# gMedAI-Lab/GAViKO

Measured on AMD Instinct MI355X. Metric: MRI volumes/sec (fwd+bwd) ViT-B/16 gaviko, 120x160x160, higher is better.
Workload: dtype bf16

## Files before the change

### gaviko_amd/csrc/gemm_bf16.hip

```cpp
#include "gemm_epilogue.hpp"

namespace gvk {

template <int BK>
__device__ __forceinline__ int swz_chunk(int row) {
  if constexpr (BK == 64) return (row >> 1) & 7;
  else return (0x78 >> (((row >> 2) & 3) * 2)) & 3;
}

template <int BM, int BN, int EPI, int BK = 64, bool DROP = false, int NS = 2, int NW = 4, bool SPLITK = false>
__global__ __launch_bounds__(64 * NW) void gemm_nt_kernel(GemmArgs p) {
  static_assert(NW == 4 || NW == 8, "4 or 8 waves");
  static_assert(!SPLITK || (NW == 4 && !DROP), "split-K is built on the 4-wave loops");
  static_assert(BK == 64, "the interleaved weight-row mapping is built for 128-byte tile rows");
  static_assert(NS >= 2 && NS <= 4, "2..4 LDS stages");
  constexpr int WM = BM / (NW / 2), WN = BN / 2;
  constexpr int MT = WM / 16, NT = WN / 16;
  constexpr int ROWB = BK * 2;
  constexpr int RPI = 1024 / ROWB;
  constexpr int CPR = ROWB / 16;
  constexpr int A_BYTES = BM * ROWB, W_BYTES = BN * ROWB, STAGE = A_BYTES + W_BYTES;
  extern __shared__ __attribute__((aligned(16))) char smem[];

  const int nwg = p.nbm * p.nbn;
  int wg;
  [[maybe_unused]] int piece = 0;
  if constexpr (SPLITK) {
    const int nu = nwg * p.ksplit;
    const int bid = blockIdx.x, xcd = bid & 7, q = nu >> 3, r = nu & 7;
    const int u = (xcd < r ? xcd * (q + 1) : r * (q + 1) + (xcd - r) * q) + (bid >> 3);
    wg = u / p.ksplit;
    piece = u - wg * p.ksplit;
  } else {
    const int bid = blockIdx.x, xcd = bid & 7, q = nwg >> 3, r = nwg & 7;
    wg = (xcd < r ? xcd * (q + 1) : r * (q + 1) + (xcd - r) * q) + (bid >> 3);
  }
  const int GROUP_M = p.group_m;
  const int gsz = GROUP_M * p.nbn;
  const int grp = wg / gsz, first_m = grp * GROUP_M;
  const int gm = min(p.nbm - first_m, GROUP_M);
  const int rem = wg - grp * gsz;
  int tile_m = first_m + rem % gm, tile_n = rem / gm;
  if (p.xcd_panels > 0) {
    tile_m = wg / p.nbn;
    tile_n = wg - tile_m * p.nbn;
  }
  const int m0 = tile_m * p.m_stride, n0 = tile_n * BN;

  const int lane = lane_id();
  const int wave = wave_id();
  const int wm = wave >> 1, wn = wave & 1;
  const int l15 = lane & 15, lq = lane >> 4;

  const bf16* __restrict__ Ag = p.A + (size_t)m0 * p.lda;
  const bf16* __restrict__ Wg = p.W + (size_t)n0 * p.ldw;
  if constexpr (SPLITK) {
    Ag += (size_t)piece * p.kt_per * BK;
    Wg += (size_t)piece * p.kt_per * BK;
  }

  auto stage = [&](int buf, int kt) {
    char* sA = smem + buf * STAGE;
    char* sW = sA + A_BYTES;
    const int k0 = kt * BK;
    const int rsub = lane / CPR, slot = lane % CPR;
#pragma unroll
    for (int r = 0; r < BM / (NW * RPI); ++r) {
      const int row = (r * NW + wave) * RPI + rsub;
      const int chunk = slot ^ swz_chunk<BK>(row);
      int srow = row;
      if constexpr (BM > 128 || 128 % BM != 0) srow = min(row, p.a_rows - 1 - m0);
      glds16(Ag + (size_t)srow * p.lda + k0 + chunk * 8, sA + (r * NW + wave) * 1024);
    }
#pragma unroll
    for (int r = 0; r < BN / (NW * RPI); ++r) {
      const int row = (r * NW + wave) * RPI + rsub;
      const int chunk = slot ^ swz_w(row);
      glds16(Wg + (size_t)row * p.ldw + k0 + chunk * 8, sW + (r * NW + wave) * 1024);
    }
  };

  f32x4 acc[MT][NT];
#pragma unroll
  for (int i = 0; i < MT; ++i)
#pragma unroll
    for (int j = 0; j < NT; ++j) acc[i][j] = f32x4{0.f, 0.f, 0.f, 0.f};

  int nt = p.K / BK;
  if constexpr (SPLITK) nt = min(p.kt_per, nt - piece * p.kt_per);
  if constexpr (BK == 64) {
#define GVK_LOAD_FRAGS(SA, SW, KS, XA, WB)                                                                  \
  {                                                                                                         \
    const int chunk_ = (KS) * 4 + lq;                                                                       \
    _Pragma("unroll") for (int i = 0; i < MT; ++i) {                                                        \
      const int row = wm * WM + i * 16 + l15;                                                               \
      XA[i] = *(const bf16x8*)((SA) + row * ROWB + ((chunk_ ^ swz_chunk<BK>(row)) << 4));                   \
    }                                                                                                       \
    _Pragma("unroll") for (int j = 0; j < NT; ++j) {                                                        \
      const int row = wn * WN + 32 * (j >> 1) + 8 * (l15 >> 2) + 4 * (j & 1) + (l15 & 3);                   \
      WB[j] = *(const bf16x8*)((SW) + row * ROWB + ((chunk_ ^ swz_w(row)) << 4));                           \
    }                                                                                                       \
  }
#define GVK_MMA(XA, WB)                                                                                      \
  _Pragma("unroll") for (int i = 0; i < MT; ++i)                                                            \
  _Pragma("unroll") for (int j = 0; j < NT; ++j)                                                            \
      acc[i][j] = __builtin_amdgcn_mfma_f32_16x16x32_bf16(WB[j], XA[i], acc[i][j], 0, 0, 0);
    bf16x8 xa0[MT], wb0[NT], xa1[MT], wb1[NT];
    constexpr int PER_TILE = BM / (NW * RPI) + BN / (NW * RPI);
    if constexpr (NS == 2) {
    stage(0, 0);
    if (nt > 1) stage(1, 1);
    if (nt > 1) __builtin_amdgcn_s_waitcnt(0x0F70 | (PER_TILE & 0xF) | ((PER_TILE >> 4) << 14));
    else __builtin_amdgcn_s_waitcnt(0x0F70);
    __builtin_amdgcn_s_barrier();
    GVK_LOAD_FRAGS(smem, smem + A_BYTES, 0, xa0, wb0)
    __builtin_amdgcn_s_waitcnt(0xC07F);
#define GVK_TILE(T, PREFETCH)                                                                               \
    {                                                                                                       \
      const int buf = (T) & 1;                                                                              \
      const char* sA = smem + buf * STAGE;                                                                  \
      const char* sW = sA + A_BYTES;                                                                        \
      GVK_LOAD_FRAGS(sA, sW, 1, xa1, wb1)                                                                   \
      __builtin_amdgcn_sched_barrier(0);                                                                    \
      GVK_MMA(xa0, wb0)                                                                                     \
      __builtin_amdgcn_sched_barrier(0);                                                                    \
      __syncthreads();     \
      if (PREFETCH) stage(buf, (T) + 2);                                                                    \
      GVK_LOAD_FRAGS(smem + (buf ^ 1) * STAGE, smem + (buf ^ 1) * STAGE + A_BYTES, 0, xa0, wb0)             \
      __builtin_amdgcn_sched_barrier(0);                                                                    \
      GVK_MMA(xa1, wb1)                                                                                     \
      __builtin_amdgcn_sched_barrier(0);                                                                    \
      __builtin_amdgcn_s_waitcnt(0xC07F);     \
    }
    int t = 0;
    for (; t < nt - 2; ++t) GVK_TILE(t, true)
    for (; t < nt; ++t) GVK_TILE(t, false)
#undef GVK_TILE
    } else {
    static_assert((NS - 1) * PER_TILE <= 63, "vmcnt is a 6-bit counter");
#pragma unroll
    for (int sgi = 0; sgi < NS; ++sgi)
      if (sgi < nt) stage(sgi, sgi);
    {
      const int ahead = min(nt, NS) - 1;
      if (ahead >= 3) __builtin_amdgcn_s_waitcnt(0x0F70 | ((3 * PER_TILE) & 0xF) | (((3 * PER_TILE) >> 4) << 14));
      else if (ahead == 2) __builtin_amdgcn_s_waitcnt(0x0F70 | ((2 * PER_TILE) & 0xF) | (((2 * PER_TILE) >> 4) << 14));
      else if (ahead == 1) __builtin_amdgcn_s_waitcnt(0x0F70 | (PER_TILE & 0xF) | ((PER_TILE >> 4) << 14));
      else __builtin_amdgcn_s_waitcnt(0x0F70);
    }
    __builtin_amdgcn_s_barrier();
    GVK_LOAD_FRAGS(smem, smem + A_BYTES, 0, xa0, wb0)
    __builtin_amdgcn_s_waitcnt(0xC07F);
#define GVK_TILE3(T, BUF, PREFETCH, AHEAD, LAST)                                                            \
    {                                                                                                       \
      const int buf = (BUF);                                                                                \
      const int nxt = buf == NS - 1 ? 0 : buf + 1;                                                          \
      const char* sA = smem + buf * STAGE;                                                                  \
      const char* sW = sA + A_BYTES;                                                                        \
      GVK_LOAD_FRAGS(sA, sW, 1, xa1, wb1)                                                                   \
      __builtin_amdgcn_sched_barrier(0);                                                                    \
      GVK_MMA(xa0, wb0)                                                                                     \
      __builtin_amdgcn_sched_barrier(0);                                                                    \
       \
      __builtin_amdgcn_s_waitcnt(0x0070 | (((AHEAD) * PER_TILE) & 0xF) | ((((AHEAD) * PER_TILE) >> 4) << 14)); \
      __builtin_amdgcn_s_barrier();                                                                         \
      if (PREFETCH) stage(buf, (T) + NS);                                                                   \
      if (!(LAST)) GVK_LOAD_FRAGS(smem + nxt * STAGE, smem + nxt * STAGE + A_BYTES, 0, xa0, wb0)            \
      __builtin_amdgcn_sched_barrier(0);                                                                    \
      GVK_MMA(xa1, wb1)                                                                                     \
      __builtin_amdgcn_sched_barrier(0);                                                                    \
      __builtin_amdgcn_s_waitcnt(0xC07F);                                                                   \
    }
    int t = 0, b = 0;
    for (; t < nt - NS; ++t) {
      GVK_TILE3(t, b, true, NS - 2, false)
      b = b == NS - 1 ? 0 : b + 1;
    }
    for (; t < nt; ++t) {
      const int r = nt - 1 - t;
      if (NS > 3 && r == 3) GVK_TILE3(t, b, false, 2, false)
      else if (r == 2) GVK_TILE3(t, b, false, 1, false)
      else if (r == 1) GVK_TILE3(t, b, false, 0, false)
      else GVK_TILE3(t, b, false, 0, true)
      b = b == NS - 1 ? 0 : b + 1;
    }
#undef GVK_TILE3
    }
#undef GVK_LOAD_FRAGS
#undef GVK_MMA
  }

  if constexpr (SPLITK) {
    const int tile_id = tile_m * p.nbn + tile_n;
    constexpr int kPiece = NW * MT * NT * 64 * 4;
    float* const base = p.sk_part + ((size_t)tile_id * p.ksplit) * kPiece;
    const __amdgpu_buffer_rsrc_t rs = __builtin_amdgcn_make_buffer_rsrc((void*)base, 0, p.ksplit * kPiece * 4, 0x00020000);
    const int off = ((wave * MT * NT) * 64 + lane) * 16;
#pragma unroll
    for (int i = 0; i < MT; ++i)
#pragma unroll
      for (int j = 0; j < NT; ++j)
        __builtin_amdgcn_raw_buffer_store_b128(__builtin_bit_cast(u32x4, acc[i][j]), rs, (piece * kPiece) * 4 + off + (i * NT + j) * 1024, 0, 16);
    int* const s_last = (int*)smem;
    asm volatile("s_waitcnt vmcnt(0)" ::: "memory");
    __syncthreads();
    if (threadIdx.x == 0) {
      const int t = __hip_atomic_fetch_add(p.sk_tick + tile_id, 1, __ATOMIC_RELAXED, __HIP_MEMORY_SCOPE_AGENT);
      const int last = (t == p.ksplit - 1) ? 1 : 0;
      if (last) {
        __builtin_amdgcn_fence(__ATOMIC_ACQUIRE, "agent");
        asm volatile("s_waitcnt vmcnt(0)" ::: "memory");
        __hip_atomic_store(p.sk_tick + tile_id, 0, __ATOMIC_RELAXED, __HIP_MEMORY_SCOPE_AGENT);
      }
      *s_last = last;
    }
    __syncthreads();
    if (!*s_last) return;
    if (p.ksplit == 2) {
      const int pc = piece ^ 1;
#pragma unroll
      for (int i = 0; i < MT; ++i)
#pragma unroll
        for (int j = 0; j < NT; ++j) acc[i][j] += *(const f32x4*)((const char*)base + (size_t)pc * kPiece * 4 + off + (i * NT + j) * 1024);
    } else {
#pragma unroll
      for (int i = 0; i < MT; ++i)
#pragma unroll
        for (int j = 0; j < NT; ++j) acc[i][j] = f32x4{0.f, 0.f, 0.f, 0.f};
      for (int pc = 0; pc < p.ksplit; ++pc) {
#pragma unroll
        for (int i = 0; i < MT; ++i)
#pragma unroll
          for (int j = 0; j < NT; ++j) acc[i][j] += *(const f32x4*)((const char*)base + (size_t)pc * kPiece * 4 + off + (i * NT + j) * 1024);
      }
    }
  }
  gemm_epilogue<EPI, DROP, MT, NT>(p, acc, m0 + wm * WM, n0 + wn * WN, l15, lq);
}

// ... 69 lines not shown
    const long t128 = (long)((a.M + 127) / 128) * (a.N / bn);
    static const int n768 = diag_env("GAVIKO_HIP_GEMM_N768") ? atoi(diag_env("GAVIKO_HIP_GEMM_N768")) : 3128;
    const int bm = (t128 >= 384) ? 128 : 64;
    tile = bm * 1000 + bn;
    if constexpr (EPI == GVK_EPI_STORE_BF16 || EPI == GVK_EPI_BIAS_GELU_BF16 || EPI == GVK_EPI_GELU_BWD_BF16) {
      static const int wide = diag_env("GAVIKO_HIP_GEMM_WIDE") ? atoi(diag_env("GAVIKO_HIP_GEMM_WIDE")) : 8;
      const long t256 = (long)((a.M + 255) / 256) * (a.N / 256);
      static const bool wide_bwd = diag_env("GAVIKO_HIP_GEMM_WIDE_BWD") == nullptr || diag_env("GAVIKO_HIP_GEMM_WIDE_BWD")[0] != '0';
      if (wide != 0 && a.N % 256 == 0 && a.drop_thresh == 0u && t256 >= wide_lo() && t256 <= 256 && (EPI != GVK_EPI_GELU_BWD_BF16 || wide_bwd))
        tile = (wide == 256 || a.K < 128) ? 256256 : 8256256;
    }
    static const long t64_hi = diag_env("GAVIKO_HIP_GEMM_T64HI") ? atol(diag_env("GAVIKO_HIP_GEMM_T64HI")) : 130;
    if (bm == 64 && bn == 128 && t128 <= 256 && a.K >= 512 && a.drop_thresh == 0u) {
      if (n768 == 3128) {
        long best = -1; int best_bm = 128;
        for (int cand : {128, 96, 64}) {
          const long tiles = (long)((a.M + cand - 1) / cand) * (a.N / 128);
          const long cost = ((tiles + 255) / 256) * (cand + 128);
          if (best < 0 || cost < best) { best = cost; best_bm = cand; }
        }
        static const int force_bm = diag_env("GAVIKO_HIP_GEMM_BM") ? atoi(diag_env("GAVIKO_HIP_GEMM_BM")) : 0;
        if (force_bm == 128 || force_bm == 96 || force_bm == 64) best_bm = force_bm;
        else if (t128 <= t64_hi && best_bm == 128) best_bm = 64;
        tile = best_bm == 64 ? 3064128 : best_bm == 96 ? 3096128 : 3128128;
      }
      else if (n768 == 128) tile = 128128;
      else if (n768 == 3064) tile = 3064128;
    }
  }
  if (a.drop_thresh != 0u) {
    if constexpr (EPI == GVK_EPI_BIAS_RES_F32 || EPI == GVK_EPI_BIAS_GELU_BF16 || EPI == GVK_EPI_GELU_BWD_BF16) {
      switch (tile) {
        case 128128: return launch_gemm<128, 128, EPI, true>(a, stream);
        case 128064: return launch_gemm<128, 64, EPI, true>(a, stream);
        case 64128: return launch_gemm<64, 128, EPI, true>(a, stream);
        case 64064: return launch_gemm<64, 64, EPI, true>(a, stream);
        default: return set_error(-2, "gvk_gemm_nt_bf16: unsupported tile %d", tile);
      }
    } else {
      return set_error(-2, "gvk_gemm_nt_bf16: drop_p > 0 is supported by BIAS_RES_F32, BIAS_GELU_BF16 and GELU_BWD_BF16 only");
    }
  }
  switch (tile) {
    case 8256256: return launch_gemm8p(a, EPI, 0, stream);
    case 7256256: return launch_gemm8p(a, EPI, 1, stream);
    case 2128128:
      if (a.sk_part == nullptr) return set_error(-2, "gvk_gemm_nt_bf16: tile 2128128 needs splitk_ws");
      return launch_gemm<128, 128, EPI, false, 2, 4, true>(a, stream);
    case 3128128: return launch_gemm<128, 128, EPI, false, 3>(a, stream);
    case 3064128: return launch_gemm<64, 128, EPI, false, 3>(a, stream);
    case 4064128:
      if (a.sk_part != nullptr) return launch_gemm<64, 128, EPI, false, 4, 4, true>(a, stream);
      return launch_gemm<64, 128, EPI, false, 4>(a, stream);
    case 3096128: return launch_gemm<96, 128, EPI, false, 3>(a, stream);
    case 256256:
      if constexpr (EPI == GVK_EPI_STORE_BF16 || EPI == GVK_EPI_BIAS_GELU_BF16 || EPI == GVK_EPI_GELU_BWD_BF16) return launch_gemm<256, 256, EPI, false, 2, 8>(a, stream);
      else return set_error(-2, "gvk_gemm_nt_bf16: the 256x256 tile is built for STORE_BF16, BIAS_GELU_BF16 and GELU_BWD_BF16");
    case 128128: return launch_gemm<128, 128, EPI>(a, stream);
    case 128064: return launch_gemm<128, 64, EPI>(a, stream);
    case 64128: return launch_gemm<64, 128, EPI>(a, stream);
    case 64064: return launch_gemm<64, 64, EPI>(a, stream);
    default: return set_error(-2, "gvk_gemm_nt_bf16: unsupported tile %d", tile);
  }
}

}

extern "C" int gvk_gemm_stat_parts(int N) { return N / 64; }

extern "C" int gvk_gemm_nt_bf16(const gvk_gemm_desc* d, void* stream) {
  using namespace gvk;
  GVK_REQUIRE(d != nullptr, "gvk_gemm_nt_bf16: null descriptor");
  GVK_REQUIRE(d->a && d->w && d->M > 0 && d->N > 0 && d->K > 0, "gvk_gemm_nt_bf16: null operand or empty shape");
  GVK_REQUIRE(d->K % 64 == 0, "gvk_gemm_nt_bf16: K=%d must be a multiple of 64", d->K);
  GVK_REQUIRE(d->N % 64 == 0, "gvk_gemm_nt_bf16: N=%d must be a multiple of 64", d->N);
  GVK_REQUIRE(d->lda >= d->K && d->ldw >= d->K && d->lda % 8 == 0 && d->ldw % 8 == 0,
              "gvk_gemm_nt_bf16: lda/ldw must be >= K and multiples of 8");
  GVK_REQUIRE(d->ldo % 8 == 0 && d->ldo >= d->N, "gvk_gemm_nt_bf16: ldo=%d must be >= N and a multiple of 8 (16-byte row pieces)", d->ldo);
  if (d->tile != 0) {
    const int bn = d->tile % 1000;
    GVK_REQUIRE(d->tile < 1000000 || d->K % 32 == 0, "gvk_gemm_nt_bf16: K not a multiple of 32");
    GVK_REQUIRE(bn > 0 && d->N % bn == 0, "gvk_gemm_nt_bf16: N=%d not a multiple of the tile's BN", d->N);
  }
  GemmArgs a{};
  a.A = (const bf16*)d->a; a.W = (const bf16*)d->w; a.out0 = d->out0; a.out1 = d->out1;
  a.bias = d->bias; a.res = d->res; a.aux = (const bf16*)d->aux; a.pos = d->pos;
  a.M = d->M; a.N = d->N; a.K = d->K; a.lda = d->lda; a.ldw = d->ldw; a.ldo = d->ldo;
  a.ldres = d->ldres; a.ldaux = d->ldaux; a.rows_in = d->rows_in; a.rows_out = d->rows_out; a.row_off = d->row_off;
  GVK_REQUIRE(d->drop_p >= 0.f && d->drop_p < 1.f && (d->drop_p == 0.f || d->seed_ptr != nullptr), "gvk_gemm_nt_bf16: drop_p in [0,1) and a seed word");
  a.seed = d->seed; a.seed_ptr = (const unsigned long long*)d->seed_ptr; a.drop_thresh = drop_threshold_u32(d->drop_p);
  a.inv_keep = d->drop_p > 0.f ? 1.f / (1.f - d->drop_p) : 1.f;
  GVK_REQUIRE(d->scale_cols == 0 || (d->epilogue == GVK_EPI_STORE_BF16 && d->scale_cols > 0 && d->scale_cols % 8 == 0 && d->scale_cols <= d->N),
              "gvk_gemm_nt_bf16: scale_cols=%d needs the STORE_BF16 epilogue, a multiple of 8 and <= N", d->scale_cols);
  a.scale_cols = d->scale_cols; a.col_scale = d->col_scale;
  GVK_REQUIRE(d->ln_mean == nullptr || (d->epilogue == GVK_EPI_STORE_BF16 && d->ln_rstd && d->ln_c1 && d->bias),
              "gvk_gemm_nt_bf16: the LayerNorm fold needs the STORE_BF16 epilogue, ln_rstd, ln_c1 and bias (= sum_c beta[c] W[n][c])");
  a.ln_mean = d->ln_mean; a.ln_rstd = d->ln_rstd; a.ln_c1 = d->ln_c1;
  GVK_REQUIRE(d->stat_part == nullptr || (d->epilogue == GVK_EPI_BIAS_RES_F32_BF16 && d->N % 128 == 0 && (d->tile == 0 || d->tile % 1000 == 128)),
              "gvk_gemm_nt_bf16: stat_part needs the BIAS_RES_F32_BF16 epilogue on 128-column tiles (64-column groups)");
  a.stat_part = d->stat_part; a.stat_pivot = d->stat_pivot;
  GVK_REQUIRE((d->m_panels == 0 && d->m_stride == 0) || (d->m_panels > 0 && d->m_stride > 0 && d->epilogue != GVK_EPI_PATCH_F32),
              "gvk_gemm_nt_bf16: m_panels=%d / m_stride=%d: both positive (or both 0), not with the PATCH epilogue", d->m_panels, d->m_stride);
  a.m_stride = d->m_stride; a.nbm = d->m_panels;
  GVK_REQUIRE(d->splitk_ws == nullptr || ((d->m_panels > 0 || d->tile == 2128128) && ((uintptr_t)d->splitk_ws & 255) == 0),
              "gvk_gemm_nt_bf16: splitk_ws goes with strided row panels or tile 2128128 (256-byte aligned)");
  GVK_REQUIRE(d->ksplit >= 0 && d->ksplit <= 8 && (d->ksplit == 0 || d->splitk_ws != nullptr), "gvk_gemm_nt_bf16: ksplit=%d: 0 (auto) .. 8, with splitk_ws", d->ksplit);
// ... 39 lines not shown
```

### gaviko_amd/csrc/gemm_epilogue.hpp

```cpp
#pragma once
#include "common.hpp"
#include "dropout.hpp"
#include "../../include/gaviko_hip.h"

namespace gvk {

struct GemmArgs {
  const bf16* A;
  const bf16* W;
  void* out0;
  void* out1;
  const float* bias;
  const float* res;
  const bf16* aux;
  const float* pos;
  int M, N, K, lda, ldw, ldo, ldres, ldaux;
  int rows_in, rows_out, row_off;
  int nbm, nbn;
  int group_m;
  int xcd_panels;
  int a_rows;
  int m_stride;
  int ksplit, kt_per;
  float* sk_part;
  int* sk_tick;
  size_t sk_bytes;
  unsigned long long seed; const unsigned long long* seed_ptr; unsigned int drop_thresh; float inv_keep;
  int scale_cols; float col_scale;
  const float* ln_mean; const float* ln_rstd; const float* ln_c1;
  float* stat_part;
  const float* stat_pivot;
  int aux_grad;
};

__device__ __forceinline__ int swz_a128(int row) { return (row >> 1) & 7; }
__device__ __forceinline__ int swz_w(int row) { return ((row >> 1) & 1) | (((row >> 3) & 3) << 1); }

template <int EPI, bool DROP, int MT, int NT>
__device__ __forceinline__ void gemm_epilogue(const GemmArgs& p, f32x4 (&acc)[MT][NT], const int mbase, const int nbase, const int l15, const int lq) {
  static_assert(NT % 2 == 0, "tile pairs");
  constexpr int NP = NT / 2;
  constexpr bool kRes = EPI == GVK_EPI_BIAS_RES_F32 || EPI == GVK_EPI_BIAS_RES_F32_BF16;
  constexpr bool kAux = EPI == GVK_EPI_GELU_BWD_BF16 || EPI == GVK_EPI_RELU_BWD_BF16;
  constexpr bool kPos = EPI == GVK_EPI_PATCH_F32;
  constexpr bool kFold = EPI == GVK_EPI_STORE_BF16;
  constexpr bool kStat = EPI == GVK_EPI_BIAS_RES_F32_BF16;
  f32x4 bv[NP][2];
  [[maybe_unused]] f32x4 c1v[NP][2];
#pragma unroll
  for (int jp = 0; jp < NP; ++jp) {
    bv[jp][0] = bv[jp][1] = f32x4{0.f, 0.f, 0.f, 0.f};
    const int n = nbase + 32 * jp + 8 * lq;
    if (p.bias != nullptr) {
      bv[jp][0] = *(const f32x4*)(p.bias + n);
      bv[jp][1] = *(const f32x4*)(p.bias + n + 4);
    }
    if constexpr (kFold) {
      c1v[jp][0] = c1v[jp][1] = f32x4{0.f, 0.f, 0.f, 0.f};
      if (p.ln_mean != nullptr) {
        c1v[jp][0] = *(const f32x4*)(p.ln_c1 + n);
        c1v[jp][1] = *(const f32x4*)(p.ln_c1 + n + 4);
      }
    }
  }
  struct Side { f32x4 r0[NP], r1[NP]; bf16x8 a8[NP]; float mu, rs, pv; };
  auto fetch = [&](const int i, Side& sd) {
    const int m = mbase + i * 16 + l15;
    if (m >= p.M) return;
    if constexpr (kFold) {
      if (p.ln_mean != nullptr) { sd.mu = p.ln_mean[m]; sd.rs = p.ln_rstd[m]; }
    }
    if constexpr (kStat) sd.pv = p.stat_pivot != nullptr ? p.stat_pivot[m] : 0.f;
#pragma unroll
    for (int jp = 0; jp < NP; ++jp) {
      const int n = nbase + 32 * jp + 8 * lq;
      if constexpr (kRes) {
        const float* rp = p.res + (size_t)m * p.ldres + n;
        sd.r0[jp] = *(const f32x4*)rp;
        sd.r1[jp] = *(const f32x4*)(rp + 4);
      } else if constexpr (kPos) {
        const float* pp = p.pos + (size_t)(m % p.rows_in) * p.N + n;
        sd.r0[jp] = *(const f32x4*)pp;
        sd.r1[jp] = *(const f32x4*)(pp + 4);
      } else if constexpr (kAux) {
        sd.a8[jp] = *(const bf16x8*)(p.aux + (size_t)m * p.ldaux + n);
      }
    }
  };
  Side cur, nxt;
  fetch(0, cur);
#pragma unroll
  for (int i = 0; i < MT; ++i) {
    if (i + 1 < MT) fetch(i + 1, nxt);
    const int m = mbase + i * 16 + l15;
    [[maybe_unused]] float ps1 = 0.f, ps2 = 0.f;
    if (m < p.M) {
      size_t orow = (size_t)m;
      if constexpr (kPos) {
        const int s = m / p.rows_in;
        orow = (size_t)s * p.rows_out + p.row_off + (m - s * p.rows_in);
      }
#pragma unroll
      for (int jp = 0; jp < NP; ++jp) {
        const int n = nbase + 32 * jp + 8 * lq;
        float v[8];
#pragma unroll
        for (int e = 0; e < 4; ++e) { v[e] = acc[i][2 * jp][e] + bv[jp][0][e]; v[4 + e] = acc[i][2 * jp + 1][e] + bv[jp][1][e]; }
        if constexpr (kFold) {
          if (p.ln_mean != nullptr) {
#pragma unroll
            for (int e = 0; e < 4; ++e) {
              v[e] = __builtin_fmaf(__builtin_fmaf(-cur.mu, c1v[jp][0][e], acc[i][2 * jp][e]), cur.rs, bv[jp][0][e]);
              v[4 + e] = __builtin_fmaf(__builtin_fmaf(-cur.mu, c1v[jp][1][e], acc[i][2 * jp + 1][e]), cur.rs, bv[jp][1][e]);
            }
          }
        }
        auto store_f32 = [&](float* dst) {
          *(f32x4*)dst = f32x4{v[0], v[1], v[2], v[3]};
          *(f32x4*)(dst + 4) = f32x4{v[4], v[5], v[6], v[7]};
        };
        auto store_bf16 = [&](bf16* dst) {
          bf16x8 o;
#pragma unroll
          for (int e = 0; e < 8; ++e) o[e] = (bf16)v[e];
          *(bf16x8*)dst = o;
        };
        [[maybe_unused]] auto drop8 = [&]() {
          const unsigned long long sd = p.seed + *p.seed_ptr;
#pragma unroll
          for (int e = 0; e < 8; ++e) v[e] *= drop_scale(sd, (unsigned long long)m * p.N + n + e, p.drop_thresh, p.inv_keep);
        };
        if constexpr (EPI == GVK_EPI_STORE_BF16) {
          if (n < p.scale_cols) {
#pragma unroll
            for (int e = 0; e < 8; ++e) v[e] *= p.col_scale;
          }
          store_bf16((bf16*)p.out0 + (size_t)m * p.ldo + n);
        } else if constexpr (kRes) {
          if constexpr (DROP) drop8();
#pragma unroll
          for (int e = 0; e < 4; ++e) { v[e] += cur.r0[jp][e]; v[4 + e] += cur.r1[jp][e]; }
          store_f32((float*)p.out0 + (size_t)m * p.ldo + n);
          if constexpr (EPI == GVK_EPI_BIAS_RES_F32_BF16) {
            store_bf16((bf16*)p.out1 + (size_t)m * p.ldo + n);
#pragma unroll
            for (int e = 0; e < 8; ++e) { const float dv = v[e] - cur.pv; ps1 += dv; ps2 = __builtin_fmaf(dv, dv, ps2); }
          }
        } else if constexpr (EPI == GVK_EPI_BIAS_GELU_BF16) {
          if (p.aux_grad != 0) {
            bf16x8 g8;
#pragma unroll
            for (int e = 0; e < 8; ++e) {
              float y, dy;
              gelu_fast_both(v[e], y, dy);
              v[e] = y;
              g8[e] = (bf16)dy;
            }
            *(bf16x8*)((bf16*)p.out0 + (size_t)m * p.ldo + n) = g8;
          } else {
            if (p.out0 != nullptr) store_bf16((bf16*)p.out0 + (size_t)m * p.ldo + n);
#pragma unroll
            for (int e = 0; e < 8; ++e) v[e] = gelu_fast(v[e]);
          }
          if constexpr (DROP) drop8();
          store_bf16((bf16*)p.out1 + (size_t)m * p.ldo + n);
        } else if constexpr (kPos) {
#pragma unroll
          for (int e = 0; e < 4; ++e) { v[e] += cur.r0[jp][e]; v[4 + e] += cur.r1[jp][e]; }
          store_f32((float*)p.out0 + orow * p.ldo + n);
          if (p.out1 != nullptr) store_f32((float*)p.out1 + (size_t)m * p.ldo + n);
        } else if constexpr (EPI == GVK_EPI_GELU_BWD_BF16) {
          if constexpr (DROP) drop8();
#pragma unroll
          for (int e = 0; e < 8; ++e) v[e] *= p.aux_grad != 0 ? (float)cur.a8[jp][e] : gelu_fast_grad((float)cur.a8[jp][e]);
          store_bf16((bf16*)p.out0 + (size_t)m * p.ldo + n);
        } else if constexpr (EPI == GVK_EPI_STORE_F32) {
          store_f32((float*)p.out0 + (size_t)m * p.ldo + n);
        } else if constexpr (EPI == GVK_EPI_BIAS_RELU_BF16) {
#pragma unroll
          for (int e = 0; e < 8; ++e) v[e] = fmaxf(v[e], 0.f);
          store_bf16((bf16*)p.out0 + (size_t)m * p.ldo + n);
        } else if constexpr (EPI == GVK_EPI_RELU_BWD_BF16) {
#pragma unroll
          for (int e = 0; e < 8; ++e) v[e] = (float)cur.a8[jp][e] > 0.f ? v[e] : 0.f;
          store_bf16((bf16*)p.out0 + (size_t)m * p.ldo + n);
        }
      }
    }
    if constexpr (kStat) {
      if (p.stat_part != nullptr) {
        ps1 += __shfl_xor(ps1, 16, 64); ps2 += __shfl_xor(ps2, 16, 64);
        ps1 += __shfl_xor(ps1, 32, 64); ps2 += __shfl_xor(ps2, 32, 64);
        if (lq == 0 && m < p.M) *(f32x2*)(p.stat_part + ((size_t)(nbase / (16 * NT)) * p.M + m) * 2) = f32x2{ps1, ps2};
      }
    }
    cur = nxt;
  }
}

int launch_gemm8p(const GemmArgs& a, int epilogue, int variant, hipStream_t stream);
bool gemm8p_supports(int epilogue);

}
```

### gaviko_amd/engine.py

```python
from __future__ import annotations

import os
from typing import Dict, List, Optional

import torch

from . import lib as L
from . import ops
from .engine_analysis import AnalysisPaths
from .engine_common import (GRAPH_WARMUP, PLAN_TIMING, SEED_EMB, SEED_LAYER, SEED_PROMPT, USE_GRAPHS, _ABLATE, _EPI_NAMES, _SIDE_STREAMS, Names,
                            _on, flat_views)
from .engine_common import evp_highpass_operator
from .engine_gaviko import GavikoPaths
from .engine_peft import PeftPaths

GEMM_MARKS = None


_BB_KINDS = ("vit", "adaptformer", "gaviko", "dvpt", "evp", "vpt", "ssf")


class Engine(GavikoPaths, PeftPaths, AnalysisPaths):
    def __init__(self, kind: str, cfg: dict, params: Dict[str, torch.nn.Parameter], depth, heads, dim, mlp_dim):
        self.kind, self.cfg, self.p = kind, cfg, params
        self.depth, self.heads, self.C, self.mlp = depth, heads, dim, mlp_dim
        self.lora_layers = frozenset(cfg.get("lora_layer") or range(depth)) if kind == "melo" else frozenset()
        self.names = Names(kind, self.lora_layers if kind == "melo" else None)
        fp, ip = cfg["frame_patch_size"], cfg["image_patch_size"]
        self.patch = (fp, ip, ip)
        self.grid = (cfg["frames"] // fp, cfg["image_size"] // ip, cfg["image_size"] // ip)
        self.N = self.grid[0] * self.grid[1] * self.grid[2]
        self.Kp = fp * ip * ip
        self.K = cfg["num_classes"]
        prec = str(cfg.get("precision") or os.environ.get("GAVIKO_HIP_PRECISION", "bf16")).lower()
        if prec not in ("bf16", "fp32", "float32"):
            raise L.GavikoHipError(f"precision={prec!r}: expected 'bf16' or 'fp32'")
        self.fp32 = prec != "bf16"
        self.q_scale = 64 ** -0.5 * ops.LOG2E
        self.adt = torch.float32 if self.fp32 else torch.bfloat16
        if cfg.get("dim_head", 64) != 64:
            raise L.GavikoHipError("the attention kernels are built for dim_head = 64")
        if cfg.get("channels", 1) != 1:
            raise L.GavikoHipError("patch embedding is built for single-channel volumes (channels = 1)")
        self.pool = cfg.get("pool", "cls")
        if kind == "gaviko":
            self.P = cfg["num_prompts"]
            self.Lat = cfg.get("prompt_latent_dim", 20)
            if cfg.get("local_dim", 20) != self.Lat:
                raise L.GavikoHipError("local_dim and prompt_latent_dim must match (one latent width per build)")
            self.share = cfg.get("share_factor", 1)
            self.T = self.P + 1 + self.N
            self.row_off = self.P + 1
            dhw = cfg.get("DHW", (10, 10, 10))
            if dhw is None:
                self.win = tuple(2 * g + 1 for g in self.grid)
            else:
                if tuple(dhw) != self.grid:
                    raise L.GavikoHipError(f"DHW={tuple(dhw)} does not match the patch grid {self.grid}")
                self.win = tuple(cfg.get("local_k", (3, 6, 6)))
        elif kind == "evp":
            self.P, self.T, self.row_off = 0, 1 + self.N, 1
            self.r = dim // int(cfg.get("scale_factor", 32))
            widths = [w_ for w_ in (4, 8, 16, 20, 24, 32) if w_ >= self.r]
            if not widths or self.r < 1:
                raise L.GavikoHipError(f"EVP: prompt rank dim/scale_factor = {self.r} is outside the rank-L kernels' range (1..32)")
            self.Lp = widths[0]
            self.freq = float(cfg.get("freq_nums", 0.25))
        elif kind == "dvpt":
            self.P = cfg.get("num_prompts", 50)
# ... 17 lines not shown
            if self.Ts[-1] <= 1 + self.pd:
                raise L.GavikoHipError("deep VPT: the shrinking sequence runs out of tokens for this depth / prompt_dim")
        self._w16: Dict[str, torch.Tensor] = {}
        self._w16_version = None
        self._shadowed = frozenset(self._backbone_weight_names())
        self._fwd_gen = 0
        self.static_io = False
        self._have_dgrad = False
        self._graphs = {}
        self._calls = {}
        self._wss = {}
        self._streams = {}
        self._recording = False
        self._keep_inputs = False
        self._eff: Dict[str, torch.Tensor] = {}
        self._fuse_proj = (kind == "gaviko" and not self.fp32 and ops.rowproj_supported(self.Lat, dim)
                           and L.diag_env("GAVIKO_HIP_FUSE_PROJ", "1") != "0")
        self.prune_dead_rows = kind == "gaviko" and not self.fp32 and os.environ.get("GAVIKO_HIP_PRUNE", "1") != "0"
        self._dy16 = kind == "gaviko" and not self.fp32 and L.diag_env("GAVIKO_HIP_DY16", "1") != "0"
        self._gelu_grad = kind == "gaviko" and not self.fp32 and L.diag_env("GAVIKO_HIP_GELU_GRAD", "1") != "0"
        self._fuse_local = kind == "gaviko" and ops.side_tile_supported(self.Lat, dim)
        self._fuse_bnd = self._fuse_local and L.diag_env("GAVIKO_HIP_FUSE_BOUNDARY", "1") != "0"
        self._fuse_next = self._fuse_local and L.diag_env("GAVIKO_HIP_FUSE_NEXT", "1") != "0"
        self._mwsa_pending = None
        self._pgrad = (kind == "gaviko" and ops.param_grads_supported(cfg.get("prompt_latent_dim", 20), dim)
                       and L.diag_env("GAVIKO_HIP_PGRAD", "1") != "0")
        self._fuse_up = (kind == "gaviko" and not self.fp32 and 3 * self.Lat + 2 <= 64 and L.diag_env("GAVIKO_HIP_FUSE_UP", "1") != "0")
        self.ldx = self.mlp + 64 if self._fuse_up else self.mlp
        self._fold_ln1 = (self._fuse_up and self._fuse_proj and dim % 128 == 0 and L.diag_env("GAVIKO_HIP_FOLD_LN1", "1") != "0")
        self._fold: Dict[str, torch.Tensor] = {}
        self._fold_version = None
        self._fold_names = frozenset(self._fold_deps()) if self._fold_ln1 else frozenset()
        self._fold_on = False
        self._marks = []
        self.plan_marks = {}
        self._bucket_marks = {}
        self.plan_bucket_marks = {}
        self._want_bucket_marks = False
        self._gemm_marks = []
        self.plan_gemm_marks = {}
        self._ws = None
        self._step = 0
        self._flat_grad = None
        self._flat_names = None
        self.bucket_layers = 4
        self._saved = None
        self._pre_is_grad = False
        self._relv = None
        self._igrad = None
        self._ig_scratch = {}
        self._conv_t_version = None

    def _gemm(self, a, w, M, out0, alg_k=None, **kw):
        if GEMM_MARKS is None or not self._recording:
            return ops.gemm_nt(a, w, M, out0, **kw)
        N, K = w.shape[0], int(kw.get("K") or w.shape[1])
        ka = int(alg_k) if alg_k is not None else K
        key = f"gemm_nt_{'f32' if self.fp32 else 'bf16'}[{_EPI_NAMES[kw['epilogue']]}] M={M} N={N} K={K}"
        mrows = M
        if kw.get("m_panels"):
            mrows = 64 * kw["m_panels"]
            key += f" panels={kw['m_panels']}x64"
        cur = torch.cuda.current_stream()
        e0 = self._ev_record(cur)
        ops.gemm_nt(a, w, M, out0, **kw)
        e1 = self._ev_record(cur)
        self._gemm_marks.append((key, 2.0 * mrows * N * ka, [mrows, N, K], None, e0, e1))

    def collect_gemm_marks(self, acc=None):
        import ctypes
        acc = {} if acc is None else acc
        lib, ms = L.load(), ctypes.c_float()
        for pid, marks in self.plan_gemm_marks.items():
            overhead = 0.0
            for key, flops, shape, nbytes, e0, e1 in marks:
                L.check(lib.gvk_plan_event_elapsed(pid, e0, e1, ctypes.byref(ms)), "gvk_plan_event_elapsed")
                if key == "__empty__":
                    overhead = ms.value
                    continue
                rec = acc.setdefault(key, {"ms": [], "flops": flops, "shape": shape, "bytes": nbytes, "overhead_ms": overhead})
                rec["ms"].append(ms.value)
        return acc

    def _d(self, name) -> torch.Tensor:
        eff = self._eff.get(name)
        return self.p[name].detach() if eff is None else eff

    def _backbone_weight_names(self) -> List[str]:
        n = [self.names.conv() + ".weight"]
        for i in range(self.depth):
            n += [self.names.qkv_weight(i), self.names.attn(i) + ".to_out.0.weight", self.names.mlp(i) + ".net.1.weight",
                  self.names.mlp(i) + ".net.4.weight"]
        return n

    def refresh_weights(self, need_dgrad: bool) -> None:
        if self.kind == "ssf":
            return
        names = self._backbone_weight_names()
        version = tuple(self.p[n]._version for n in names) + tuple(self.p[n].data_ptr() for n in names)
        stale = version != self._w16_version
        w = self._w16
        if stale:
            conv = self._d(names[0]).reshape(self.C, self.Kp).contiguous()
            w["conv"] = ops.to_operand(conv, None if self.fp32 else w.get("conv"), self.adt)
        if not stale and (not need_dgrad or self._have_dgrad):
            return
# ... 915 lines not shown
```

Baseline: 771.4.

## Add narrow-N 64xBN GEMM tiles for few-panel GEMMs to raise workgroup count

Generalizes the bf16 NT GEMM kernel to support 64/32/16-column tiles. It adds a 1-wide wave-N layout, a single-tile weight swizzle, uneven weight slabs with per-wave vmcnt waits, and a half-width epilogue. The engine now auto-selects these narrow tiles for panelled GEMMs with fewer than 16 panels, so small-M GEMMs launch more workgroups and fill more CUs. The cost is less operand reuse per tile, and the new uneven-slab and swizzle paths add risk.

```diff
diff --git a/gaviko_amd/csrc/gemm_bf16.hip b/gaviko_amd/csrc/gemm_bf16.hip
--- a/gaviko_amd/csrc/gemm_bf16.hip
+++ b/gaviko_amd/csrc/gemm_bf16.hip
@@ -14,12 +14,17 @@
   static_assert(!SPLITK || (NW == 4 && !DROP), "split-K is built on the 4-wave loops");
   static_assert(BK == 64, "the interleaved weight-row mapping is built for 128-byte tile rows");
   static_assert(NS >= 2 && NS <= 4, "2..4 LDS stages");
-  constexpr int WM = BM / (NW / 2), WN = BN / 2;
+  constexpr int WAVES_N = BN >= 64 ? 2 : 1, WAVES_M = NW / WAVES_N;
+  constexpr int WM = BM / WAVES_M, WN = BN / WAVES_N;
+  static_assert(WM % 16 == 0 && WN % 16 == 0, "whole 16 x 16 MFMA tiles per wave");
   constexpr int MT = WM / 16, NT = WN / 16;
+  static_assert(NT == 1 || NT % 2 == 0, "tile pairs, or the single 16-column tile");
   constexpr int ROWB = BK * 2;
   constexpr int RPI = 1024 / ROWB;
   constexpr int CPR = ROWB / 16;
   constexpr int A_BYTES = BM * ROWB, W_BYTES = BN * ROWB, STAGE = A_BYTES + W_BYTES;
+  constexpr int W_FULL = BN / (NW * RPI), W_REM = (BN / RPI) % NW;
+  static_assert(BN % RPI == 0 && (W_REM == 0 || (NS >= 3 && !SPLITK)), "uneven weight slabs: the counted-vmcnt loop only");
   extern __shared__ __attribute__((aligned(16))) char smem[];
 
   const int nwg = p.nbm * p.nbn;
@@ -49,7 +54,8 @@
 
   const int lane = lane_id();
   const int wave = wave_id();
-  const int wm = wave >> 1, wn = wave & 1;
+  const int wm = wave / WAVES_N, wn = wave % WAVES_N;
+  auto swz_wt = [](const int row) { return NT == 1 ? swz_a128(row) : swz_w(row); };
   const int l15 = lane & 15, lq = lane >> 4;
 
   const bf16* __restrict__ Ag = p.A + (size_t)m0 * p.lda;
@@ -73,10 +79,17 @@
       glds16(Ag + (size_t)srow * p.lda + k0 + chunk * 8, sA + (r * NW + wave) * 1024);
     }
 #pragma unroll
-    for (int r = 0; r < BN / (NW * RPI); ++r) {
+    for (int r = 0; r < W_FULL; ++r) {
       const int row = (r * NW + wave) * RPI + rsub;
-      const int chunk = slot ^ swz_w(row);
+      const int chunk = slot ^ swz_wt(row);
       glds16(Wg + (size_t)row * p.ldw + k0 + chunk * 8, sW + (r * NW + wave) * 1024);
+    }
+    if constexpr (W_REM != 0) {
+      if (wave < W_REM) {
+        const int row = (W_FULL * NW + wave) * RPI + rsub;
+        const int chunk = slot ^ swz_wt(row);
+        glds16(Wg + (size_t)row * p.ldw + k0 + chunk * 8, sW + (W_FULL * NW + wave) * 1024);
+      }
     }
   };
 
@@ -97,8 +110,8 @@
       XA[i] = *(const bf16x8*)((SA) + row * ROWB + ((chunk_ ^ swz_chunk<BK>(row)) << 4));                   \
     }                                                                                                       \
     _Pragma("unroll") for (int j = 0; j < NT; ++j) {                                                        \
-      const int row = wn * WN + 32 * (j >> 1) + 8 * (l15 >> 2) + 4 * (j & 1) + (l15 & 3);                   \
-      WB[j] = *(const bf16x8*)((SW) + row * ROWB + ((chunk_ ^ swz_w(row)) << 4));                           \
+      const int row = NT == 1 ? wn * WN + l15 : wn * WN + 32 * (j >> 1) + 8 * (l15 >> 2) + 4 * (j & 1) + (l15 & 3); \
+      WB[j] = *(const bf16x8*)((SW) + row * ROWB + ((chunk_ ^ swz_wt(row)) << 4));                          \
     }                                                                                                       \
   }
 #define GVK_MMA(XA, WB)                                                                                      \
@@ -106,7 +119,7 @@
   _Pragma("unroll") for (int j = 0; j < NT; ++j)                                                            \
       acc[i][j] = __builtin_amdgcn_mfma_f32_16x16x32_bf16(WB[j], XA[i], acc[i][j], 0, 0, 0);
     bf16x8 xa0[MT], wb0[NT], xa1[MT], wb1[NT];
-    constexpr int PER_TILE = BM / (NW * RPI) + BN / (NW * RPI);
+    constexpr int PER_TILE = BM / (NW * RPI) + W_FULL;
     if constexpr (NS == 2) {
     stage(0, 0);
     if (nt > 1) stage(1, 1);
@@ -137,15 +150,21 @@
     for (; t < nt; ++t) GVK_TILE(t, false)
 #undef GVK_TILE
     } else {
-    static_assert((NS - 1) * PER_TILE <= 63, "vmcnt is a 6-bit counter");
+    static_assert((NS - 1) * (PER_TILE + (W_REM != 0)) <= 63, "vmcnt is a 6-bit counter");
+#define GVK_WAIT_TILES(BASE, TILES)                                                                         \
+    {                                                                                                       \
+      constexpr int c0_ = (TILES) * PER_TILE, c1_ = (TILES) * (PER_TILE + 1);                               \
+      if (W_REM != 0 && wave < W_REM) __builtin_amdgcn_s_waitcnt((BASE) | (c1_ & 0xF) | ((c1_ >> 4) << 14)); \
+      else __builtin_amdgcn_s_waitcnt((BASE) | (c0_ & 0xF) | ((c0_ >> 4) << 14));                           \
+    }
 #pragma unroll
     for (int sgi = 0; sgi < NS; ++sgi)
       if (sgi < nt) stage(sgi, sgi);
     {
       const int ahead = min(nt, NS) - 1;
-      if (ahead >= 3) __builtin_amdgcn_s_waitcnt(0x0F70 | ((3 * PER_TILE) & 0xF) | (((3 * PER_TILE) >> 4) << 14));
-      else if (ahead == 2) __builtin_amdgcn_s_waitcnt(0x0F70 | ((2 * PER_TILE) & 0xF) | (((2 * PER_TILE) >> 4) << 14));
-      else if (ahead == 1) __builtin_amdgcn_s_waitcnt(0x0F70 | (PER_TILE & 0xF) | ((PER_TILE >> 4) << 14));
+      if (ahead >= 3) GVK_WAIT_TILES(0x0F70, 3)
+      else if (ahead == 2) GVK_WAIT_TILES(0x0F70, 2)
+      else if (ahead == 1) GVK_WAIT_TILES(0x0F70, 1)
       else __builtin_amdgcn_s_waitcnt(0x0F70);
     }
     __builtin_amdgcn_s_barrier();
@@ -162,7 +181,7 @@
       GVK_MMA(xa0, wb0)                                                                                     \
       __builtin_amdgcn_sched_barrier(0);                                                                    \
        \
-      __builtin_amdgcn_s_waitcnt(0x0070 | (((AHEAD) * PER_TILE) & 0xF) | ((((AHEAD) * PER_TILE) >> 4) << 14)); \
+      GVK_WAIT_TILES(0x0070, AHEAD)                                                                         \
       __builtin_amdgcn_s_barrier();                                                                         \
       if (PREFETCH) stage(buf, (T) + NS);                                                                   \
       if (!(LAST)) GVK_LOAD_FRAGS(smem + nxt * STAGE, smem + nxt * STAGE + A_BYTES, 0, xa0, wb0)            \
@@ -185,6 +204,7 @@
       b = b == NS - 1 ? 0 : b + 1;
     }
 #undef GVK_TILE3
+#undef GVK_WAIT_TILES
     }
 #undef GVK_LOAD_FRAGS
 #undef GVK_MMA
@@ -360,6 +380,15 @@
     case 4064128:
       if (a.sk_part != nullptr) return launch_gemm<64, 128, EPI, false, 4, 4, true>(a, stream);
       return launch_gemm<64, 128, EPI, false, 4>(a, stream);
+    case 4064064: case 4064032: case 4064016:
+      if constexpr (EPI == GVK_EPI_STORE_BF16 || EPI == GVK_EPI_BIAS_RES_F32 || EPI == GVK_EPI_BIAS_GELU_BF16 || EPI == GVK_EPI_GELU_BWD_BF16) {
+        if (a.sk_part != nullptr) return set_error(-2, "gvk_gemm_nt_bf16: tile %d has no split-K form", tile);
+        if (tile == 4064064) return launch_gemm<64, 64, EPI, false, 4>(a, stream);
+        if (tile == 4064032) return launch_gemm<64, 32, EPI, false, 4>(a, stream);
+        return launch_gemm<64, 16, EPI, false, 4>(a, stream);
+      } else {
+        return set_error(-2, "gvk_gemm_nt_bf16: tile %d is built for STORE_BF16, BIAS_RES_F32, BIAS_GELU_BF16 and GELU_BWD_BF16", tile);
+      }
     case 3096128: return launch_gemm<96, 128, EPI, false, 3>(a, stream);
     case 256256:
       if constexpr (EPI == GVK_EPI_STORE_BF16 || EPI == GVK_EPI_BIAS_GELU_BF16 || EPI == GVK_EPI_GELU_BWD_BF16) return launch_gemm<256, 256, EPI, false, 2, 8>(a, stream);
diff --git a/gaviko_amd/csrc/gemm_epilogue.hpp b/gaviko_amd/csrc/gemm_epilogue.hpp
--- a/gaviko_amd/csrc/gemm_epilogue.hpp
+++ b/gaviko_amd/csrc/gemm_epilogue.hpp
@@ -1,4 +1,5 @@
 #pragma once
+#include <type_traits>
 #include "common.hpp"
 #include "dropout.hpp"
 #include "../../include/gaviko_hip.h"
@@ -38,8 +39,12 @@
 
 template <int EPI, bool DROP, int MT, int NT>
 __device__ __forceinline__ void gemm_epilogue(const GemmArgs& p, f32x4 (&acc)[MT][NT], const int mbase, const int nbase, const int l15, const int lq) {
-  static_assert(NT % 2 == 0, "tile pairs");
-  constexpr int NP = NT / 2;
+  static_assert(NT == 1 || NT % 2 == 0, "tile pairs, or the single 16-column tile");
+  constexpr int H = NT == 1 ? 1 : 2;
+  constexpr int PW = 4 * H;
+  constexpr int NP = NT / H;
+  using auxv = std::conditional_t<H == 2, bf16x8, bf16x4>;
+  auto col = [&](const int jp) { return H == 2 ? nbase + 32 * jp + 8 * lq : nbase + 4 * lq; };
   constexpr bool kRes = EPI == GVK_EPI_BIAS_RES_F32 || EPI == GVK_EPI_BIAS_RES_F32_BF16;
   constexpr bool kAux = EPI == GVK_EPI_GELU_BWD_BF16 || EPI == GVK_EPI_RELU_BWD_BF16;
   constexpr bool kPos = EPI == GVK_EPI_PATCH_F32;
@@ -50,20 +55,20 @@
 #pragma unroll
   for (int jp = 0; jp < NP; ++jp) {
     bv[jp][0] = bv[jp][1] = f32x4{0.f, 0.f, 0.f, 0.f};
-    const int n = nbase + 32 * jp + 8 * lq;
+    const int n = col(jp);
     if (p.bias != nullptr) {
       bv[jp][0] = *(const f32x4*)(p.bias + n);
-      bv[jp][1] = *(const f32x4*)(p.bias + n + 4);
+      if constexpr (H == 2) bv[jp][1] = *(const f32x4*)(p.bias + n + 4);
     }
     if constexpr (kFold) {
       c1v[jp][0] = c1v[jp][1] = f32x4{0.f, 0.f, 0.f, 0.f};
       if (p.ln_mean != nullptr) {
         c1v[jp][0] = *(const f32x4*)(p.ln_c1 + n);
-        c1v[jp][1] = *(const f32x4*)(p.ln_c1 + n + 4);
+        if constexpr (H == 2) c1v[jp][1] = *(const f32x4*)(p.ln_c1 + n + 4);
       }
     }
   }
-  struct Side { f32x4 r0[NP], r1[NP]; bf16x8 a8[NP]; float mu, rs, pv; };
+  struct Side { f32x4 r0[NP], r1[NP]; auxv a8[NP]; float mu, rs, pv; };
   auto fetch = [&](const int i, Side& sd) {
     const int m = mbase + i * 16 + l15;
     if (m >= p.M) return;
@@ -73,17 +78,17 @@
     if constexpr (kStat) sd.pv = p.stat_pivot != nullptr ? p.stat_pivot[m] : 0.f;
 #pragma unroll
     for (int jp = 0; jp < NP; ++jp) {
-      const int n = nbase + 32 * jp + 8 * lq;
+      const int n = col(jp);
       if constexpr (kRes) {
         const float* rp = p.res + (size_t)m * p.ldres + n;
         sd.r0[jp] = *(const f32x4*)rp;
-        sd.r1[jp] = *(const f32x4*)(rp + 4);
+        if constexpr (H == 2) sd.r1[jp] = *(const f32x4*)(rp + 4);
       } else if constexpr (kPos) {
         const float* pp = p.pos + (size_t)(m % p.rows_in) * p.N + n;
         sd.r0[jp] = *(const f32x4*)pp;
-        sd.r1[jp] = *(const f32x4*)(pp + 4);
+        if constexpr (H == 2) sd.r1[jp] = *(const f32x4*)(pp + 4);
       } else if constexpr (kAux) {
-        sd.a8[jp] = *(const bf16x8*)(p.aux + (size_t)m * p.ldaux + n);
+        sd.a8[jp] = *(const auxv*)(p.aux + (size_t)m * p.ldaux + n);
       }
     }
   };
@@ -102,87 +107,90 @@
       }
 #pragma unroll
       for (int jp = 0; jp < NP; ++jp) {
-        const int n = nbase + 32 * jp + 8 * lq;
-        float v[8];
-#pragma unroll
-        for (int e = 0; e < 4; ++e) { v[e] = acc[i][2 * jp][e] + bv[jp][0][e]; v[4 + e] = acc[i][2 * jp + 1][e] + bv[jp][1][e]; }
+        const int n = col(jp);
+        float v[PW];
+#pragma unroll
+        for (int e = 0; e < 4; ++e) {
+          v[e] = acc[i][H * jp][e] + bv[jp][0][e];
+          if constexpr (H == 2) v[4 + e] = acc[i][2 * jp + 1][e] + bv[jp][1][e];
+        }
         if constexpr (kFold) {
           if (p.ln_mean != nullptr) {
 #pragma unroll
             for (int e = 0; e < 4; ++e) {
-              v[e] = __builtin_fmaf(__builtin_fmaf(-cur.mu, c1v[jp][0][e], acc[i][2 * jp][e]), cur.rs, bv[jp][0][e]);
-              v[4 + e] = __builtin_fmaf(__builtin_fmaf(-cur.mu, c1v[jp][1][e], acc[i][2 * jp + 1][e]), cur.rs, bv[jp][1][e]);
+              v[e] = __builtin_fmaf(__builtin_fmaf(-cur.mu, c1v[jp][0][e], acc[i][H * jp][e]), cur.rs, bv[jp][0][e]);
+              if constexpr (H == 2) v[4 + e] = __builtin_fmaf(__builtin_fmaf(-cur.mu, c1v[jp][1][e], acc[i][2 * jp + 1][e]), cur.rs, bv[jp][1][e]);
             }
           }
         }
         auto store_f32 = [&](float* dst) {
           *(f32x4*)dst = f32x4{v[0], v[1], v[2], v[3]};
-          *(f32x4*)(dst + 4) = f32x4{v[4], v[5], v[6], v[7]};
+          if constexpr (H == 2) *(f32x4*)(dst + 4) = f32x4{v[4], v[5], v[6], v[7]};
         };
         auto store_bf16 = [&](bf16* dst) {
-          bf16x8 o;
-#pragma unroll
-          for (int e = 0; e < 8; ++e) o[e] = (bf16)v[e];
-          *(bf16x8*)dst = o;
+          auxv o;
+#pragma unroll
+          for (int e = 0; e < PW; ++e) o[e] = (bf16)v[e];
+          *(auxv*)dst = o;
         };
         [[maybe_unused]] auto drop8 = [&]() {
           const unsigned long long sd = p.seed + *p.seed_ptr;
 #pragma unroll
-          for (int e = 0; e < 8; ++e) v[e] *= drop_scale(sd, (unsigned long long)m * p.N + n + e, p.drop_thresh, p.inv_keep);
+          for (int e = 0; e < PW; ++e) v[e] *= drop_scale(sd, (unsigned long long)m * p.N + n + e, p.drop_thresh, p.inv_keep);
         };
         if constexpr (EPI == GVK_EPI_STORE_BF16) {
           if (n < p.scale_cols) {
 #pragma unroll
-            for (int e = 0; e < 8; ++e) v[e] *= p.col_scale;
+            for (int e = 0; e < PW; ++e) v[e] *= p.col_scale;
           }
           store_bf16((bf16*)p.out0 + (size_t)m * p.ldo + n);
         } else if constexpr (kRes) {
           if constexpr (DROP) drop8();
 #pragma unroll
-          for (int e = 0; e < 4; ++e) { v[e] += cur.r0[jp][e]; v[4 + e] += cur.r1[jp][e]; }
+          for (int e = 0; e < 4; ++e) { v[e] += cur.r0[jp][e]; if constexpr (H == 2) v[4 + e] += cur.r1[jp][e]; }
           store_f32((float*)p.out0 + (size_t)m * p.ldo + n);
           if constexpr (EPI == GVK_EPI_BIAS_RES_F32_BF16) {
             store_bf16((bf16*)p.out1 + (size_t)m * p.ldo + n);
 #pragma unroll
-            for (int e = 0; e < 8; ++e) { const float dv = v[e] - cur.pv; ps1 += dv; ps2 = __builtin_fmaf(dv, dv, ps2); }
+            for (int e = 0; e < PW; ++e) { const float dv = v[e] - cur.pv; ps1 += dv; ps2 = __builtin_fmaf(dv, dv, ps2); }
           }
         } else if constexpr (EPI == GVK_EPI_BIAS_GELU_BF16) {
           if (p.aux_grad != 0) {
-            bf16x8 g8;
-#pragma unroll
-            for (int e = 0; e < 8; ++e) {
+            auxv g8;
+#pragma unroll
+            for (int e = 0; e < PW; ++e) {
               float y, dy;
               gelu_fast_both(v[e], y, dy);
               v[e] = y;
               g8[e] = (bf16)dy;
             }
-            *(bf16x8*)((bf16*)p.out0 + (size_t)m * p.ldo + n) = g8;
+            *(auxv*)((bf16*)p.out0 + (size_t)m * p.ldo + n) = g8;
           } else {
             if (p.out0 != nullptr) store_bf16((bf16*)p.out0 + (size_t)m * p.ldo + n);
 #pragma unroll
-            for (int e = 0; e < 8; ++e) v[e] = gelu_fast(v[e]);
+            for (int e = 0; e < PW; ++e) v[e] = gelu_fast(v[e]);
           }
           if constexpr (DROP) drop8();
           store_bf16((bf16*)p.out1 + (size_t)m * p.ldo + n);
         } else if constexpr (kPos) {
 #pragma unroll
-          for (int e = 0; e < 4; ++e) { v[e] += cur.r0[jp][e]; v[4 + e] += cur.r1[jp][e]; }
+          for (int e = 0; e < 4; ++e) { v[e] += cur.r0[jp][e]; if constexpr (H == 2) v[4 + e] += cur.r1[jp][e]; }
           store_f32((float*)p.out0 + orow * p.ldo + n);
           if (p.out1 != nullptr) store_f32((float*)p.out1 + (size_t)m * p.ldo + n);
         } else if constexpr (EPI == GVK_EPI_GELU_BWD_BF16) {
           if constexpr (DROP) drop8();
 #pragma unroll
-          for (int e = 0; e < 8; ++e) v[e] *= p.aux_grad != 0 ? (float)cur.a8[jp][e] : gelu_fast_grad((float)cur.a8[jp][e]);
+          for (int e = 0; e < PW; ++e) v[e] *= p.aux_grad != 0 ? (float)cur.a8[jp][e] : gelu_fast_grad((float)cur.a8[jp][e]);
           store_bf16((bf16*)p.out0 + (size_t)m * p.ldo + n);
         } else if constexpr (EPI == GVK_EPI_STORE_F32) {
           store_f32((float*)p.out0 + (size_t)m * p.ldo + n);
         } else if constexpr (EPI == GVK_EPI_BIAS_RELU_BF16) {
 #pragma unroll
-          for (int e = 0; e < 8; ++e) v[e] = fmaxf(v[e], 0.f);
+          for (int e = 0; e < PW; ++e) v[e] = fmaxf(v[e], 0.f);
           store_bf16((bf16*)p.out0 + (size_t)m * p.ldo + n);
         } else if constexpr (EPI == GVK_EPI_RELU_BWD_BF16) {
 #pragma unroll
-          for (int e = 0; e < 8; ++e) v[e] = (float)cur.a8[jp][e] > 0.f ? v[e] : 0.f;
+          for (int e = 0; e < PW; ++e) v[e] = (float)cur.a8[jp][e] > 0.f ? v[e] : 0.f;
           store_bf16((bf16*)p.out0 + (size_t)m * p.ldo + n);
         }
       }
diff --git a/gaviko_amd/engine.py b/gaviko_amd/engine.py
--- a/gaviko_amd/engine.py
+++ b/gaviko_amd/engine.py
@@ -15,6 +15,17 @@
 from .engine_peft import PeftPaths
 
 GEMM_MARKS = None
+
+_NARROW_PANEL_EPIS = (ops.EPI_STORE_BF16, ops.EPI_BIAS_RES_F32, ops.EPI_BIAS_GELU_BF16, ops.EPI_GELU_BWD_BF16)
+
+
+def panel_tile(panels: int, N: int) -> int:
+    if panels >= 16:
+        return 0
+    for bn in (32, 64):
+        if N % bn == 0 and panels * (N // bn) <= 768:
+            return 4064000 + bn
+    return 0
 
 
 _BB_KINDS = ("vit", "adaptformer", "gaviko", "dvpt", "evp", "vpt", "ssf")
@@ -138,6 +149,8 @@
         self._conv_t_version = None
 
     def _gemm(self, a, w, M, out0, alg_k=None, **kw):
+        if kw.get("m_panels") and not kw.get("tile") and not self.fp32 and not kw.get("drop_p") and kw["epilogue"] in _NARROW_PANEL_EPIS:
+            kw["tile"] = panel_tile(kw["m_panels"], int(kw.get("N") or w.shape[0]))
         if GEMM_MARKS is None or not self._recording:
             return ops.gemm_nt(a, w, M, out0, **kw)
         N, K = w.shape[0], int(kw.get("K") or w.shape[1])
```

After: 770.8. No clear change (-0.1%).
